# yilundu/cross_attention_renderer

Hardware: AMD Instinct MI355X
Metric: rendered_rays_per_sec (higher is better)
Workload: dtype f32 (split-f16 x3 MFMA); 1 GPU; 256x256 query frame, 64 samples/view, 2 context views (config 2), a new query pose every step (cameras on the host), 1 forward call(s) x 1 scene(s) x 65536 rays per rank; builder_kept=False, H=256, samples_per_view=64, parallelism=one GPU

## Files before the change

cross_attention_renderer_amd/csrc/car_raychain.hip:

```cpp
#include "car_common.h"
#include "car_geom.h"

namespace {

#include "car_mma32.h"
#include "car_lds_dma.h"
#include "car_fused_layout.h"
#include "car_chain_layout.h"

struct Chunk { unsigned off; int nt; };
struct ChainArgs {
    const float* arena;
    const float* bias;
    const float* scale;
    int layer[kMaxLayers];
    Chunk chunk[kMaxChunks];
    int n_chunks;
    const float* x0; int ld0;
    const float* x1; int ld1;
    const float* z1_in;
    float* out0;
    float* out1;
    const CarRay* rays;
    long M;
    int V, R;
    float zscale;
};

struct Stream {
    const ChainArgs& a;
    float* lds;
    int g;
    __device__ __forceinline__ float* buffer(int gi) const { return lds + (gi % kRing) * kBufFloats; }
    __device__ __forceinline__ void issue(int gi, int tid, int wave) const {
        if (gi >= a.n_chunks) return;
        const Chunk c = a.chunk[gi];
        const float* src = a.arena + c.off;
        float* dst = buffer(gi);
        for (int t = 0; t < c.nt; ++t) {
            const unsigned lds_dst = __builtin_amdgcn_readfirstlane((unsigned)(uintptr_t)(lds_void*)(dst + 4 * (t * 256 + wave * 64)));
            const float* gsrc = src + 4 * (t * 256 + tid);
            lds_dma16(gsrc, lds_dst);
        }
    }
    __device__ __forceinline__ void landed(int gi) const {
        const int n = __builtin_amdgcn_readfirstlane(gi + 1 < a.n_chunks ? a.chunk[gi + 1].nt : 0);
        switch (n) {
            case kTileCounts[0]: wait_vm<kTileCounts[0]>(); break;
            case kTileCounts[1]: wait_vm<kTileCounts[1]>(); break;
            case kTileCounts[2]: wait_vm<kTileCounts[2]>(); break;
            default: wait_vm<0>(); break;
        }
        __syncthreads();
    }
    __device__ __forceinline__ void sync() const { landed(g + 1); }
};

static_assert(kTileFloats == kMma32Tile && kChunkK == 32 && kTileN == 32, "the packers' tile is the one mma_chunk reads");
template <int NT>
__device__ __forceinline__ void scale(f32x16 (&acc)[NT], float f) {
#pragma unroll
    for (int t = 0; t < NT; ++t) acc[t] *= f;
}

template <int NT>
__device__ __forceinline__ void layer_global(f32x16 (&acc)[NT], const float* xrow, int K, int chunks, float dW, Stream& st, int tid, int lane,
                                             int wave) {
    const int h = lane >> 5;
    auto load = [&](int c, float (&x8)[2][8]) {
#pragma unroll
        for (int kg = 0; kg < 2; ++kg) {
            const int k0 = 32 * c + 16 * kg + 8 * h;
#pragma unroll
            for (int q = 0; q < 2; ++q) {
                const int kq = k0 + 4 * q;
                const float4 v = *reinterpret_cast<const float4*>(xrow + (kq + 4 <= K ? kq : 0));
                const float e[4] = {v.x, v.y, v.z, v.w};
#pragma unroll
                for (int i = 0; i < 4; ++i) x8[kg][4 * q + i] = kq + 4 <= K ? e[i] : (kq + i < K ? xrow[kq + i] : 0.0f);
            }
        }
    };
    float m = 0.0f;
    for (int c = 0; c < chunks; ++c) {
        float x8[2][8];
        load(c, x8);
#pragma unroll
        for (int kg = 0; kg < 2; ++kg)
#pragma unroll
            for (int e = 0; e < 8; ++e) m = fmaxf(m, fabsf(x8[kg][e]));
    }
    m = fmaxf(m, __shfl_xor(m, 32, 64));
    float p, pinv;
    pow2_scale(fmaxf(m, 1e-30f), p, pinv);
    scale<NT>(acc, p / dW);
    float cur[2][8], nxt[2][8];
    load(0, cur);
    for (int c = 0; c < chunks; ++c) {
        st.issue(st.g + 2, tid, wave);
        if (c + 1 < chunks) load(c + 1, nxt);
        mma_chunk<NT>(acc, st.buffer(st.g) + 4 * lane, cur, p);
#pragma unroll
        for (int kg = 0; kg < 2; ++kg)
#pragma unroll
            for (int e = 0; e < 8; ++e) cur[kg][e] = nxt[kg][e];
        st.sync();
        ++st.g;
    }
    scale<NT>(acc, dW * pinv);
}
template <int NSRC, int NT, bool RELU>
__device__ __forceinline__ void layer_chained(f32x16 (&acc)[NT], const f32x16 (&src)[NSRC], float dW, Stream& st, int tid, int lane, int wave) {
    float m = 0.0f;
#pragma unroll
    for (int T = 0; T < NSRC; ++T)
#pragma unroll
        for (int r = 0; r < 16; ++r) m = fmaxf(m, RELU ? src[T][r] : fabsf(src[T][r]));
    m = fmaxf(m, __shfl_xor(m, 32, 64));
    float p, pinv;
    pow2_scale(fmaxf(m, 1e-30f), p, pinv);
    scale<NT>(acc, p / dW);
#pragma unroll
    for (int T = 0; T < NSRC; ++T) {
        st.issue(st.g + 2, tid, wave);
        float x8[2][8];
#pragma unroll
        for (int kg = 0; kg < 2; ++kg)
#pragma unroll
            for (int e = 0; e < 8; ++e) x8[kg][e] = RELU ? fmaxf(src[T][8 * kg + e], 0.0f) : src[T][8 * kg + e];
        mma_chunk<NT>(acc, st.buffer(st.g) + 4 * lane, x8, p);
        st.sync();
        ++st.g;
    }
    scale<NT>(acc, dW * pinv);
}
template <int NT>
__device__ __forceinline__ void store_rows(const f32x16 (&acc)[NT], float* row, int N, int h) {
#pragma unroll
    for (int t = 0; t < NT; ++t)
#pragma unroll
        for (int g = 0; g < 4; ++g) {
            const int n0 = mma32_channel(t, 4 * g, h);
            if (n0 + 4 <= N) *reinterpret_cast<float4*>(row + n0) = make_float4(acc[t][4 * g], acc[t][4 * g + 1], acc[t][4 * g + 2], acc[t][4 * g + 3]);
        }
}

static_assert(chain_tiles(kSlotLatentValue) == 9 && chain_tiles(kSlotEncodeLatent) == 4 && chain_tiles(kSlotQueryRepeat) == 4 &&
              chain_tiles(kSlotLinIn) == 4 && chain_tiles(chain_block_slot(0, 0)) == 4 && chain_tiles(chain_block_slot(0, 1)) == 4 &&
              chain_tiles(chain_block_slot(0, 2)) == 4 && chain_tiles(kSlotLinOut) == 1, "the kernels' <9>, <4>, <1> are the table's tile counts");
static_assert(tail_block_bias(0, 0) == kTailBiasLinIn + kD && tail_block_bias(0, 2) == kTailBiasLinIn + 3 * kD && tail_block_bias(1, 0) == kTailBiasLinIn + 4 * kD &&
              tail_block_pos(0, 2) == kTailPosBlocks + 2 && tail_block_pos(1, 0) == kTailPosBlocks + 3, "the tail's spelled-out offsets and positions");
constexpr int kLvK = kChainLayer[kSlotLatentValue].K, kLvChunks = chain_chunks(kSlotLatentValue);
constexpr int kInK = kChainLayer[kSlotLinIn].K, kInChunks = chain_chunks(kSlotLinIn);
__global__ void __launch_bounds__(256, 1) ray_mid_kernel(const ChainArgs a) {
    extern __shared__ __attribute__((aligned(16))) float lds[];
    const int tid = threadIdx.x, lane = tid & 63, wave = tid >> 6, s = lane & 31, h = lane >> 5;
    const long row = (long)blockIdx.x * 128 + wave * 32 + s;
    const long lrow = row < a.M ? row : a.M - 1;
    auto dW = [&](int i) { return a.scale[kMaxLayers + a.layer[i]]; };
    Stream st{a, lds, 0};
    st.issue(0, tid, wave);
    st.issue(1, tid, wave);
    st.landed(0);
    f32x16 z1[9];
    zero<9>(z1);
    add_bias<9>(z1, a.bias, h);
    layer_global<9>(z1, a.x0 + lrow * a.ld0, kLvK, kLvChunks, dW(0), st, tid, lane, wave);
    if (row < a.M) store_rows<9>(z1, a.out0 + row * kE, kE, h);
    f32x16 hb[4];
    zero<4>(hb);
    add_bias<4>(hb, a.bias + kMidBiasEncodeLatent, h);
    layer_chained<9, 4, false>(hb, z1, dW(1), st, tid, lane, wave);
    f32x16 uh[4];
    zero<4>(uh);
    layer_chained<4, 4, false>(uh, hb, dW(2), st, tid, lane, wave);
    if (row < a.M) store_rows<4>(uh, a.out1 + row * kD, kD, h);
}

__global__ void __launch_bounds__(256, 1) ray_tail_kernel(const ChainArgs a) {
    extern __shared__ __attribute__((aligned(16))) float lds[];
    const int tid = threadIdx.x, lane = tid & 63, wave = tid >> 6, s = lane & 31, h = lane >> 5;
    const long row = (long)blockIdx.x * 128 + wave * 32 + s;
    const long lrow = row < a.M ? row : a.M - 1;
    auto dW = [&](int i) { return a.scale[kMaxLayers + a.layer[i]]; };
    Stream st{a, lds, 0};
    st.issue(0, tid, wave);
    st.issue(1, tid, wave);
    st.landed(0);
    f32x16 z[9];
#pragma unroll
    for (int t = 0; t < 9; ++t)
#pragma unroll
        for (int g = 0; g < 4; ++g) {
            const float4 v = row4(a.z1_in + lrow * kE, t, g, h);
            z[t][4 * g] = a.zscale * v.x; z[t][4 * g + 1] = a.zscale * v.y; z[t][4 * g + 2] = a.zscale * v.z; z[t][4 * g + 3] = a.zscale * v.w;
        }
    add_bias<9>(z, a.bias, h);
    layer_global<9>(z, a.x0 + lrow * a.ld0, kLvK, kLvChunks, dW(0), st, tid, lane, wave);
    const float* bias = a.bias + kTailBiasLinIn;
    f32x16 x[4], net[4];
    zero<4>(x);
    add_bias<4>(x, bias, h);
    layer_global<4>(x, a.x1 + lrow * a.ld1, kInK, kInChunks, dW(1), st, tid, lane, wave);
#pragma unroll
    for (int i = 0; i < kBlocks; ++i) {
        add_bias<4>(x, bias + (3 * i + 1) * kD, h);
        layer_chained<9, 4, false>(x, z, dW(kTailPosBlocks + 0 + 3 * i), st, tid, lane, wave);
        zero<4>(net);
        add_bias<4>(net, bias + (3 * i + 2) * kD, h);
        layer_chained<4, 4, true>(net, x, dW(kTailPosBlocks + 1 + 3 * i), st, tid, lane, wave);
        add_bias<4>(x, bias + (3 * i + 3) * kD, h);
        layer_chained<4, 4, true>(x, net, dW(kTailPosBlocks + 2 + 3 * i), st, tid, lane, wave);
    }
    f32x16 o[1];
    zero<1>(o);
    add_bias<1>(o, bias + (kTailBiasLinOut - kTailBiasLinIn), h);
    layer_chained<4, 1, true>(o, x, dW(kTailPosLinOut), st, tid, lane, wave);
    if (row < a.M && h == 0) {
        const long sc = row / a.R, r = row % a.R;
        float ov = 0.0f;
        for (int v = 0; v < a.V; ++v) ov = fmaxf(ov, a.rays[(sc * a.V + v) * a.R + r].overlaps);
        const float valid = ov > 0.0f ? 1.0f : 0.0f;
        for (int k = 0; k < 3; ++k) a.out0[3 * row + k] = o[0][k] * valid + (1.0f - valid);
        a.out1[row] = valid;
    }
}

}

extern "C" size_t car_chain_packed_floats(int K, int N) { return chain_packed_floats(K, N); }
extern "C" int car_chain_pack(const float* W, int ldw, const float* W2, int K, int N, int chained, float* packed, float* scale, int slot,
                              void* stream) {
    CAR_REQUIRE(W && packed && scale && K > 0 && N > 0 && ldw >= K && slot >= 0 && slot < kMaxLayers, "car_chain_pack: bad arguments");
    const car_pack_scale s{nullptr, scale + slot, scale + kMaxLayers + slot};
    (void)hipGetLastError();
    car_pack_absmax((hipStream_t)stream, 1, W, ldw, W2, nullptr, N, K, s);
    car_pack_tiles32((hipStream_t)stream, 256, W, ldw, W2, N, K, chain_tiles_of(N), chain_chunks_of(K), 2, chained, s, reinterpret_cast<_Float16*>(packed));
    CAR_CHECK_LAUNCH("car_chain_pack");
    return CAR_OK;
}

namespace {
int launch_chain(bool tail, const float* arena, const unsigned* offs, const int* nts, int n_chunks, const float* bias, const float* scale,
                 const int* layers, int n_layers, const float* x0, int ld0, const float* x1, int ld1, const float* z1_in, float* out0, float* out1,
                 const float* rays, long M, int V, int R, float zscale, void* stream) {
    CAR_REQUIRE(n_chunks > 0 && n_chunks <= kMaxChunks && n_layers == (tail ? kTailLayers : kMidLayers), "car_ray_chain: %d weight chunks, %d layers", n_chunks, n_layers);
    ChainArgs a;
    a.arena = arena; a.bias = bias; a.scale = scale; a.n_chunks = n_chunks;
    for (int i = 0; i < kMaxLayers; ++i) a.layer[i] = i < n_layers ? layers[i] : 0;
    for (int i = 0; i < n_layers; ++i) CAR_REQUIRE(layers[i] >= 0 && layers[i] < kMaxLayers, "car_ray_chain: bad scale slot");
    for (int i = 0; i < n_chunks; ++i) {
        CAR_REQUIRE(chain_tile_count_ok(nts[i]), "car_ray_chain: chunk %d has %d tiles (1, 4 or 9)", i, nts[i]);
        a.chunk[i].off = offs[i]; a.chunk[i].nt = nts[i];
    }
    a.x0 = x0; a.ld0 = ld0; a.x1 = x1; a.ld1 = ld1; a.z1_in = z1_in; a.out0 = out0; a.out1 = out1; a.rays = (const CarRay*)rays;
    a.M = M; a.V = V; a.R = R; a.zscale = zscale;
    const size_t lds_bytes = (size_t)kRing * kBufFloats * sizeof(float);
    auto kern = tail ? ray_tail_kernel : ray_mid_kernel;
    CAR_LAUNCH_LDS("car_ray_chain", kern, dim3(car_div_up(M, 128)), dim3(256), lds_bytes, (hipStream_t)stream, a);
    return CAR_OK;
}
}

extern "C" int car_ray_mid(const float* arena, const unsigned* offs, const int* nts, int n_chunks, const float* bias, const float* scale,
                           const int* layers, int n_layers, const float* ebar, int ld_ebar, float* z1, float* uh, long M, void* stream) {
    CAR_REQUIRE(arena && offs && nts && bias && scale && layers && ebar && z1 && uh && M > 0 && ld_ebar >= kC && ld_ebar % 4 == 0,
                "car_ray_mid: bad arguments");
    return launch_chain(false, arena, offs, nts, n_chunks, bias, scale, layers, n_layers, ebar, ld_ebar, nullptr, 0, nullptr, z1, uh, nullptr, M, 0, 1,
                        0.0f, stream);
}
extern "C" int car_ray_tail(const float* arena, const unsigned* offs, const int* nts, int n_chunks, const float* bias, const float* scale,
                            const int* layers, int n_layers, const float* ebar, int ld_ebar, const float* phi_x, int ld_phi, const float* z1,
                            const float* rays, int b, int V, int R, float* rgb, float* valid, void* stream) {
    CAR_REQUIRE(arena && offs && nts && bias && scale && layers && ebar && phi_x && z1 && rays && rgb && valid, "car_ray_tail: null pointer");
    CAR_REQUIRE(b > 0 && V > 0 && R > 0 && ld_ebar >= kC && ld_ebar % 4 == 0 && ld_phi >= kPhiLd && ld_phi % 4 == 0, "car_ray_tail: bad sizes");
    return launch_chain(true, arena, offs, nts, n_chunks, bias, scale, layers, n_layers, ebar, ld_ebar, phi_x, ld_phi, z1, rgb, valid, rays, (long)b * R, V,
                        R, (float)V, stream);
}
```

Baseline: 2.230 million rays/s.

## Switch ray chain kernels to 16x16x32 f16 MFMA tiles with eight-wave blocks

Reworks the per-ray MLP chain kernels from 32-wide MFMA tiles (32 rays per wave, 4 waves) to 16x16x32 f16 MFMA tiles with 16 rays per wave and 8 waves per block. Weight chunk streaming into LDS is split into 256-float pieces spread across the eight waves, with matching per-wave counted waits. Chained-layer operands are rebuilt with permlane32 swaps, and bias plus scaling are folded into a final step. The intent is more waves per CU and better latency hiding for the same weight stream, at the cost of more MFMA instructions per ray and a changed block size and grid.

Result: no change. 2.247 million rays/s (median of 6 runs) (+0.8%).

```diff
diff --git a/cross_attention_renderer_amd/csrc/car_raychain.hip b/cross_attention_renderer_amd/csrc/car_raychain.hip
--- a/cross_attention_renderer_amd/csrc/car_raychain.hip
+++ b/cross_attention_renderer_amd/csrc/car_raychain.hip
@@ -3,9 +3,9 @@
 
 namespace {
 
-#include "car_mma32.h"
-#include "car_lds_dma.h"
-#include "car_fused_layout.h"
+constexpr int kWaves = 8;
+constexpr int kWaveRays = 16, kGroupRays = kWaves * kWaveRays;
+#include "car_mma_tile.h"
 #include "car_chain_layout.h"
 
 struct Chunk { unsigned off; int nt; };
@@ -27,196 +27,228 @@
     float zscale;
 };
 
+constexpr int kPieceFloats = 256;
+constexpr int kTilePieces = kTileFloats / kPieceFloats;
+__device__ __forceinline__ constexpr int chunk_pieces(int nt, int wave) {
+    return wave < kTilePieces * nt ? (kTilePieces * nt - wave + kWaves - 1) / kWaves : 0;
+}
+static_assert(chunk_pieces(kMaxNT, 0) <= 5, "Stream::landed has counted waits for up to five pieces per wave");
+
 struct Stream {
     const ChainArgs& a;
     float* lds;
     int g;
     __device__ __forceinline__ float* buffer(int gi) const { return lds + (gi % kRing) * kBufFloats; }
-    __device__ __forceinline__ void issue(int gi, int tid, int wave) const {
+    __device__ __forceinline__ void issue(int gi, int lane, int wave) const {
         if (gi >= a.n_chunks) return;
         const Chunk c = a.chunk[gi];
         const float* src = a.arena + c.off;
         float* dst = buffer(gi);
-        for (int t = 0; t < c.nt; ++t) {
-            const unsigned lds_dst = __builtin_amdgcn_readfirstlane((unsigned)(uintptr_t)(lds_void*)(dst + 4 * (t * 256 + wave * 64)));
-            const float* gsrc = src + 4 * (t * 256 + tid);
-            lds_dma16(gsrc, lds_dst);
-        }
-    }
-    __device__ __forceinline__ void landed(int gi) const {
-        const int n = __builtin_amdgcn_readfirstlane(gi + 1 < a.n_chunks ? a.chunk[gi + 1].nt : 0);
+        const int n = kTilePieces * c.nt;
+        for (int kb = wave; kb < n; kb += kWaves) {
+            const unsigned lds_dst = __builtin_amdgcn_readfirstlane((unsigned)(uintptr_t)(lds_void*)(dst + kb * kPieceFloats));
+            lds_dma16(src + kb * kPieceFloats, 16u * (unsigned)lane, lds_dst);
+        }
+    }
+    __device__ __forceinline__ void landed(int gi, int wave) const {
+        const int n = __builtin_amdgcn_readfirstlane(gi + 1 < a.n_chunks ? chunk_pieces(a.chunk[gi + 1].nt, wave) : 0);
         switch (n) {
-            case kTileCounts[0]: wait_vm<kTileCounts[0]>(); break;
-            case kTileCounts[1]: wait_vm<kTileCounts[1]>(); break;
-            case kTileCounts[2]: wait_vm<kTileCounts[2]>(); break;
+            case 1: wait_vm<1>(); break;
+            case 2: wait_vm<2>(); break;
+            case 3: wait_vm<3>(); break;
+            case 4: wait_vm<4>(); break;
+            case 5: wait_vm<5>(); break;
             default: wait_vm<0>(); break;
         }
         __syncthreads();
     }
-    __device__ __forceinline__ void sync() const { landed(g + 1); }
+    __device__ __forceinline__ void sync(int wave) const { landed(g + 1, wave); }
 };
 
-static_assert(kTileFloats == kMma32Tile && kChunkK == 32 && kTileN == 32, "the packers' tile is the one mma_chunk reads");
+static_assert(kTileFloats == 2 * kTile && kChunkK == 32 && kTileN == 32, "a packed tile holds two 16-output tiles of a K = 32 step: [kg][hi | lo][lane][8 halves]");
+__device__ __forceinline__ int a_offset(int lane) {
+    const int q = lane >> 4;
+    return (q >> 1) * (kTileFloats / 2) + 4 * ((lane & 15) + 32 * (q & 1));
+}
+constexpr int kAhead = 3;
 template <int NT>
-__device__ __forceinline__ void scale(f32x16 (&acc)[NT], float f) {
-#pragma unroll
-    for (int t = 0; t < NT; ++t) acc[t] *= f;
-}
-
+__device__ __forceinline__ void mma_chunk(f32x4 (&acc)[NT], const float* wl, const half8& bhi, const half8& blo) {
+    static_assert(NT % 2 == 0, "two 16-output tiles per packed tile");
+    half8 ah[kAhead + 1], al[kAhead + 1];
+    auto read = [&](int t) {
+        const float* w = wl + (t >> 1) * kTileFloats + (t & 1) * (4 * 16);
+        ah[t % (kAhead + 1)] = __builtin_bit_cast(half8, *reinterpret_cast<const float4*>(w));
+        al[t % (kAhead + 1)] = __builtin_bit_cast(half8, *reinterpret_cast<const float4*>(w + kTile / 2));
+    };
+#pragma unroll
+    for (int t = 0; t < kAhead && t < NT; ++t) read(t);
+#pragma unroll
+    for (int t = 0; t < NT; ++t) {
+        if (t + kAhead < NT) read(t + kAhead);
+        __builtin_amdgcn_sched_barrier(0);
+        const int s = t % (kAhead + 1);
+        acc[t] = __builtin_amdgcn_mfma_f32_16x16x32_f16(ah[s], bhi, acc[t], 0, 0, 0);
+        acc[t] = __builtin_amdgcn_mfma_f32_16x16x32_f16(ah[s], blo, acc[t], 0, 0, 0);
+        acc[t] = __builtin_amdgcn_mfma_f32_16x16x32_f16(al[s], bhi, acc[t], 0, 0, 0);
+        __builtin_amdgcn_sched_barrier(0);
+    }
+}
 template <int NT>
-__device__ __forceinline__ void layer_global(f32x16 (&acc)[NT], const float* xrow, int K, int chunks, float dW, Stream& st, int tid, int lane,
-                                             int wave) {
-    const int h = lane >> 5;
-    auto load = [&](int c, float (&x8)[2][8]) {
-#pragma unroll
-        for (int kg = 0; kg < 2; ++kg) {
-            const int k0 = 32 * c + 16 * kg + 8 * h;
-#pragma unroll
-            for (int q = 0; q < 2; ++q) {
-                const int kq = k0 + 4 * q;
-                const float4 v = *reinterpret_cast<const float4*>(xrow + (kq + 4 <= K ? kq : 0));
-                const float e[4] = {v.x, v.y, v.z, v.w};
-#pragma unroll
-                for (int i = 0; i < 4; ++i) x8[kg][4 * q + i] = kq + 4 <= K ? e[i] : (kq + i < K ? xrow[kq + i] : 0.0f);
-            }
+__device__ __forceinline__ void zero(f32x4 (&acc)[NT]) {
+#pragma unroll
+    for (int t = 0; t < NT; ++t) acc[t] = f32x4{0.0f, 0.0f, 0.0f, 0.0f};
+}
+template <int NT>
+__device__ __forceinline__ void finish(f32x4 (&acc)[NT], float f, const float* bias, int q) {
+#pragma unroll
+    for (int t = 0; t < NT; ++t) {
+        acc[t] *= f;
+        if (bias) {
+            const float4 b4 = *reinterpret_cast<const float4*>(bias + 16 * t + 4 * q);
+            acc[t][0] += b4.x; acc[t][1] += b4.y; acc[t][2] += b4.z; acc[t][3] += b4.w;
+        }
+    }
+}
+
+template <int NT, int K, bool FRESH>
+__device__ __forceinline__ void layer_global(f32x4 (&acc)[NT], const float* xrow, float dW, const float* bias, Stream& st, int lane, int wave) {
+    constexpr int kChunks = chain_chunks_of(K);
+    const int q = lane >> 4;
+    auto load = [&](int c, float (&x8)[8]) {
+#pragma unroll
+        for (int i = 0; i < 2; ++i) {
+            const int kq = 32 * c + 8 * q + 4 * i;
+            const bool whole = K % kChunkK == 0 || kq + 4 <= K;
+            const float4 v = *reinterpret_cast<const float4*>(xrow + (whole ? kq : 0));
+            const float e[4] = {v.x, v.y, v.z, v.w};
+#pragma unroll
+            for (int r = 0; r < 4; ++r) x8[4 * i + r] = whole ? e[r] : (kq + r < K ? xrow[kq + r] : 0.0f);
         }
     };
     float m = 0.0f;
-    for (int c = 0; c < chunks; ++c) {
-        float x8[2][8];
+    for (int c = 0; c < kChunks; ++c) {
+        float x8[8];
         load(c, x8);
 #pragma unroll
-        for (int kg = 0; kg < 2; ++kg)
-#pragma unroll
-            for (int e = 0; e < 8; ++e) m = fmaxf(m, fabsf(x8[kg][e]));
-    }
+        for (int e = 0; e < 8; ++e) m = fmaxf(m, fabsf(x8[e]));
+    }
+    m = fmaxf(m, __shfl_xor(m, 16, 64));
     m = fmaxf(m, __shfl_xor(m, 32, 64));
     float p, pinv;
     pow2_scale(fmaxf(m, 1e-30f), p, pinv);
-    scale<NT>(acc, p / dW);
-    float cur[2][8], nxt[2][8];
+    if (FRESH) zero<NT>(acc);
+    else scale_acc<NT>(acc, p / dW);
+    const int ao = a_offset(lane);
+    float cur[8], nxt[8];
     load(0, cur);
-    for (int c = 0; c < chunks; ++c) {
-        st.issue(st.g + 2, tid, wave);
-        if (c + 1 < chunks) load(c + 1, nxt);
-        mma_chunk<NT>(acc, st.buffer(st.g) + 4 * lane, cur, p);
-#pragma unroll
-        for (int kg = 0; kg < 2; ++kg)
-#pragma unroll
-            for (int e = 0; e < 8; ++e) cur[kg][e] = nxt[kg][e];
-        st.sync();
+    for (int c = 0; c < kChunks; ++c) {
+        st.issue(st.g + 2, lane, wave);
+        if (c + 1 < kChunks) load(c + 1, nxt);
+        half8 bhi, blo;
+        split8(cur, p, bhi, blo);
+        mma_chunk<NT>(acc, st.buffer(st.g) + ao, bhi, blo);
+#pragma unroll
+        for (int e = 0; e < 8; ++e) cur[e] = nxt[e];
+        st.sync(wave);
         ++st.g;
     }
-    scale<NT>(acc, dW * pinv);
-}
-template <int NSRC, int NT, bool RELU>
-__device__ __forceinline__ void layer_chained(f32x16 (&acc)[NT], const f32x16 (&src)[NSRC], float dW, Stream& st, int tid, int lane, int wave) {
-    float m = 0.0f;
-#pragma unroll
-    for (int T = 0; T < NSRC; ++T)
-#pragma unroll
-        for (int r = 0; r < 16; ++r) m = fmaxf(m, RELU ? src[T][r] : fabsf(src[T][r]));
-    m = fmaxf(m, __shfl_xor(m, 32, 64));
+    finish<NT>(acc, dW * pinv, bias, q);
+}
+template <int NSRC, bool RELU>
+__device__ __forceinline__ void chained_operand(const f32x4 (&src)[NSRC], int c, float (&x8)[8]) {
+#pragma unroll
+    for (int r = 0; r < 4; ++r) {
+        const float lo = RELU ? fmaxf(src[2 * c][r], 0.0f) : src[2 * c][r], hi = RELU ? fmaxf(src[2 * c + 1][r], 0.0f) : src[2 * c + 1][r];
+        const auto sw = __builtin_amdgcn_permlane32_swap(__float_as_uint(lo), __float_as_uint(hi), false, false);
+        x8[r] = __uint_as_float(sw[0]);
+        x8[4 + r] = __uint_as_float(sw[1]);
+    }
+}
+template <int NSRC, int NT, bool RELU, bool FRESH>
+__device__ __forceinline__ void layer_chained(f32x4 (&acc)[NT], const f32x4 (&src)[NSRC], float dW, const float* bias, Stream& st, int lane, int wave) {
+    static_assert(NSRC % 2 == 0, "a K step takes two source tiles");
+    const float m = sample_max<NSRC, RELU>(src);
     float p, pinv;
     pow2_scale(fmaxf(m, 1e-30f), p, pinv);
-    scale<NT>(acc, p / dW);
-#pragma unroll
-    for (int T = 0; T < NSRC; ++T) {
-        st.issue(st.g + 2, tid, wave);
-        float x8[2][8];
-#pragma unroll
-        for (int kg = 0; kg < 2; ++kg)
-#pragma unroll
-            for (int e = 0; e < 8; ++e) x8[kg][e] = RELU ? fmaxf(src[T][8 * kg + e], 0.0f) : src[T][8 * kg + e];
-        mma_chunk<NT>(acc, st.buffer(st.g) + 4 * lane, x8, p);
-        st.sync();
+    if (FRESH) zero<NT>(acc);
+    else scale_acc<NT>(acc, p / dW);
+    const int ao = a_offset(lane);
+    half8 bhi, blo;
+    {
+        float x8[8];
+        chained_operand<NSRC, RELU>(src, 0, x8);
+        split8(x8, p, bhi, blo);
+    }
+#pragma unroll
+    for (int c = 0; c < NSRC / 2; ++c) {
+        st.issue(st.g + 2, lane, wave);
+        mma_chunk<NT>(acc, st.buffer(st.g) + ao, bhi, blo);
+        if (c + 1 < NSRC / 2) {
+            float x8[8];
+            chained_operand<NSRC, RELU>(src, c + 1, x8);
+            split8(x8, p, bhi, blo);
+        }
+        st.sync(wave);
         ++st.g;
     }
-    scale<NT>(acc, dW * pinv);
-}
-template <int NT>
-__device__ __forceinline__ void store_rows(const f32x16 (&acc)[NT], float* row, int N, int h) {
-#pragma unroll
-    for (int t = 0; t < NT; ++t)
-#pragma unroll
-        for (int g = 0; g < 4; ++g) {
-            const int n0 = mma32_channel(t, 4 * g, h);
-            if (n0 + 4 <= N) *reinterpret_cast<float4*>(row + n0) = make_float4(acc[t][4 * g], acc[t][4 * g + 1], acc[t][4 * g + 2], acc[t][4 * g + 3]);
-        }
-}
-
-static_assert(chain_tiles(kSlotLatentValue) == 9 && chain_tiles(kSlotEncodeLatent) == 4 && chain_tiles(kSlotQueryRepeat) == 4 &&
-              chain_tiles(kSlotLinIn) == 4 && chain_tiles(chain_block_slot(0, 0)) == 4 && chain_tiles(chain_block_slot(0, 1)) == 4 &&
-              chain_tiles(chain_block_slot(0, 2)) == 4 && chain_tiles(kSlotLinOut) == 1, "the kernels' <9>, <4>, <1> are the table's tile counts");
+    finish<NT>(acc, dW * pinv, bias, lane >> 4);
+}
+
+static_assert(2 * chain_tiles(kSlotLatentValue) == kTE && 2 * chain_tiles(kSlotEncodeLatent) == kTD && 2 * chain_tiles(kSlotQueryRepeat) == kTD &&
+              2 * chain_tiles(kSlotLinIn) == kTD && 2 * chain_tiles(chain_block_slot(0, 0)) == kTD && 2 * chain_tiles(chain_block_slot(0, 1)) == kTD &&
+              2 * chain_tiles(chain_block_slot(0, 2)) == kTD && chain_tiles(kSlotLinOut) == 1 && kTE == 18 && kTD == 8, "the kernels' tile counts are the table's");
 static_assert(tail_block_bias(0, 0) == kTailBiasLinIn + kD && tail_block_bias(0, 2) == kTailBiasLinIn + 3 * kD && tail_block_bias(1, 0) == kTailBiasLinIn + 4 * kD &&
               tail_block_pos(0, 2) == kTailPosBlocks + 2 && tail_block_pos(1, 0) == kTailPosBlocks + 3, "the tail's spelled-out offsets and positions");
-constexpr int kLvK = kChainLayer[kSlotLatentValue].K, kLvChunks = chain_chunks(kSlotLatentValue);
-constexpr int kInK = kChainLayer[kSlotLinIn].K, kInChunks = chain_chunks(kSlotLinIn);
-__global__ void __launch_bounds__(256, 1) ray_mid_kernel(const ChainArgs a) {
+constexpr int kLvK = kChainLayer[kSlotLatentValue].K, kInK = kChainLayer[kSlotLinIn].K;
+__global__ void __launch_bounds__(64 * kWaves) ray_mid_kernel(const ChainArgs a) {
     extern __shared__ __attribute__((aligned(16))) float lds[];
-    const int tid = threadIdx.x, lane = tid & 63, wave = tid >> 6, s = lane & 31, h = lane >> 5;
-    const long row = (long)blockIdx.x * 128 + wave * 32 + s;
+    const int tid = threadIdx.x, lane = tid & 63, wave = __builtin_amdgcn_readfirstlane(tid >> 6), q = lane >> 4;
+    const long row = (long)blockIdx.x * kGroupRays + wave * kWaveRays + (lane & 15);
     const long lrow = row < a.M ? row : a.M - 1;
     auto dW = [&](int i) { return a.scale[kMaxLayers + a.layer[i]]; };
     Stream st{a, lds, 0};
-    st.issue(0, tid, wave);
-    st.issue(1, tid, wave);
-    st.landed(0);
-    f32x16 z1[9];
-    zero<9>(z1);
-    add_bias<9>(z1, a.bias, h);
-    layer_global<9>(z1, a.x0 + lrow * a.ld0, kLvK, kLvChunks, dW(0), st, tid, lane, wave);
-    if (row < a.M) store_rows<9>(z1, a.out0 + row * kE, kE, h);
-    f32x16 hb[4];
-    zero<4>(hb);
-    add_bias<4>(hb, a.bias + kMidBiasEncodeLatent, h);
-    layer_chained<9, 4, false>(hb, z1, dW(1), st, tid, lane, wave);
-    f32x16 uh[4];
-    zero<4>(uh);
-    layer_chained<4, 4, false>(uh, hb, dW(2), st, tid, lane, wave);
-    if (row < a.M) store_rows<4>(uh, a.out1 + row * kD, kD, h);
-}
-
-__global__ void __launch_bounds__(256, 1) ray_tail_kernel(const ChainArgs a) {
+    st.issue(0, lane, wave);
+    st.issue(1, lane, wave);
+    st.landed(0, wave);
+    f32x4 z1[kTE];
+    layer_global<kTE, kLvK, true>(z1, a.x0 + lrow * a.ld0, dW(0), a.bias, st, lane, wave);
+    if (row < a.M) store_rows<kTE>(z1, a.out0 + row * kE, q);
+    f32x4 hb[kTD];
+    layer_chained<kTE, kTD, false, true>(hb, z1, dW(1), a.bias + kMidBiasEncodeLatent, st, lane, wave);
+    f32x4 uh[kTD];
+    layer_chained<kTD, kTD, false, true>(uh, hb, dW(2), nullptr, st, lane, wave);
+    if (row < a.M) store_rows<kTD>(uh, a.out1 + row * kD, q);
+}
+
+__global__ void __launch_bounds__(64 * kWaves) ray_tail_kernel(const ChainArgs a) {
     extern __shared__ __attribute__((aligned(16))) float lds[];
-    const int tid = threadIdx.x, lane = tid & 63, wave = tid >> 6, s = lane & 31, h = lane >> 5;
-    const long row = (long)blockIdx.x * 128 + wave * 32 + s;
+    const int tid = threadIdx.x, lane = tid & 63, wave = __builtin_amdgcn_readfirstlane(tid >> 6), q = lane >> 4;
+    const long row = (long)blockIdx.x * kGroupRays + wave * kWaveRays + (lane & 15);
     const long lrow = row < a.M ? row : a.M - 1;
     auto dW = [&](int i) { return a.scale[kMaxLayers + a.layer[i]]; };
     Stream st{a, lds, 0};
-    st.issue(0, tid, wave);
-    st.issue(1, tid, wave);
-    st.landed(0);
-    f32x16 z[9];
-#pragma unroll
-    for (int t = 0; t < 9; ++t)
-#pragma unroll
-        for (int g = 0; g < 4; ++g) {
-            const float4 v = row4(a.z1_in + lrow * kE, t, g, h);
-            z[t][4 * g] = a.zscale * v.x; z[t][4 * g + 1] = a.zscale * v.y; z[t][4 * g + 2] = a.zscale * v.z; z[t][4 * g + 3] = a.zscale * v.w;
-        }
-    add_bias<9>(z, a.bias, h);
-    layer_global<9>(z, a.x0 + lrow * a.ld0, kLvK, kLvChunks, dW(0), st, tid, lane, wave);
+    st.issue(0, lane, wave);
+    st.issue(1, lane, wave);
+    st.landed(0, wave);
+    f32x4 z[kTE];
+#pragma unroll
+    for (int t = 0; t < kTE; ++t) {
+        const float4 v = *reinterpret_cast<const float4*>(a.z1_in + lrow * kE + 16 * t + 4 * q);
+        z[t] = f32x4{a.zscale * v.x, a.zscale * v.y, a.zscale * v.z, a.zscale * v.w};
+    }
+    layer_global<kTE, kLvK, false>(z, a.x0 + lrow * a.ld0, dW(0), a.bias, st, lane, wave);
     const float* bias = a.bias + kTailBiasLinIn;
-    f32x16 x[4], net[4];
-    zero<4>(x);
-    add_bias<4>(x, bias, h);
-    layer_global<4>(x, a.x1 + lrow * a.ld1, kInK, kInChunks, dW(1), st, tid, lane, wave);
+    f32x4 x[kTD], net[kTD];
+    layer_global<kTD, kInK, true>(x, a.x1 + lrow * a.ld1, dW(1), bias, st, lane, wave);
 #pragma unroll
     for (int i = 0; i < kBlocks; ++i) {
-        add_bias<4>(x, bias + (3 * i + 1) * kD, h);
-        layer_chained<9, 4, false>(x, z, dW(kTailPosBlocks + 0 + 3 * i), st, tid, lane, wave);
-        zero<4>(net);
-        add_bias<4>(net, bias + (3 * i + 2) * kD, h);
-        layer_chained<4, 4, true>(net, x, dW(kTailPosBlocks + 1 + 3 * i), st, tid, lane, wave);
-        add_bias<4>(x, bias + (3 * i + 3) * kD, h);
-        layer_chained<4, 4, true>(x, net, dW(kTailPosBlocks + 2 + 3 * i), st, tid, lane, wave);
-    }
-    f32x16 o[1];
-    zero<1>(o);
-    add_bias<1>(o, bias + (kTailBiasLinOut - kTailBiasLinIn), h);
-    layer_chained<4, 1, true>(o, x, dW(kTailPosLinOut), st, tid, lane, wave);
-    if (row < a.M && h == 0) {
+        layer_chained<kTE, kTD, false, false>(x, z, dW(kTailPosBlocks + 0 + 3 * i), bias + (3 * i + 1) * kD, st, lane, wave);
+        layer_chained<kTD, kTD, true, true>(net, x, dW(kTailPosBlocks + 1 + 3 * i), bias + (3 * i + 2) * kD, st, lane, wave);
+        layer_chained<kTD, kTD, true, false>(x, net, dW(kTailPosBlocks + 2 + 3 * i), bias + (3 * i + 3) * kD, st, lane, wave);
+    }
+    f32x4 o[2];
+    layer_chained<kTD, 2, true, true>(o, x, dW(kTailPosLinOut), bias + (kTailBiasLinOut - kTailBiasLinIn), st, lane, wave);
+    if (row < a.M && q == 0) {
         const long sc = row / a.R, r = row % a.R;
         float ov = 0.0f;
         for (int v = 0; v < a.V; ++v) ov = fmaxf(ov, a.rays[(sc * a.V + v) * a.R + r].overlaps);
@@ -257,7 +289,7 @@
     a.M = M; a.V = V; a.R = R; a.zscale = zscale;
     const size_t lds_bytes = (size_t)kRing * kBufFloats * sizeof(float);
     auto kern = tail ? ray_tail_kernel : ray_mid_kernel;
-    CAR_LAUNCH_LDS("car_ray_chain", kern, dim3(car_div_up(M, 128)), dim3(256), lds_bytes, (hipStream_t)stream, a);
+    CAR_LAUNCH_LDS("car_ray_chain", kern, dim3(car_div_up(M, kGroupRays)), dim3(64 * kWaves), lds_bytes, (hipStream_t)stream, a);
     return CAR_OK;
 }
 }
```
